# shaunliewsmu/ai-laryngeal-video-based-classifier

Measured on AMD Instinct MI355X. Metric: clips/sec fwd ViViT-B 32x224^2 bf16, higher is better.
Workload: dtype bf16; 1 GPU; ViViT-B/16x2 forward, 32x224x224 clips, batch 8 per GPU (BASELINE configs[1]); model=ViViT-B/16x2 (joint space-time, 12L, d768, 12H, 3137 tokens), global_batch=8, seq_len=3137, parallelism=dp1, streams=2, hip_graph=True

## Files before the change

ai-laryngeal-video-based-classifier_amd/csrc/attention.hip:

```cpp
#include "common.hpp"

#include <type_traits>

namespace vc {

constexpr int AK = 64;
constexpr int KV_TILE_BYTES = AK * 64 * 2;
constexpr int KV_SLOT = 2 * KV_TILE_BYTES;
constexpr int NSLOT = 4;
constexpr float LIM = 256.0f;

#ifndef VC_ATTN_SWEXP
#define VC_ATTN_SWEXP 0
#endif
__device__ __forceinline__ float sw_exp2(float x) {
    x = fmaxf(x, -126.0f);
    const float t = x + 12582912.0f;
    const float f = x - (t - 12582912.0f);
    float p = __builtin_fmaf(f, 0.0550292665f, 0.2422569819f);
    p = __builtin_fmaf(f, p, 0.6932530550f);
    p = __builtin_fmaf(f, p, 0.9999513387f);
    return __builtin_bit_cast(float, __builtin_bit_cast(unsigned, p) + (__builtin_bit_cast(unsigned, t) << 23));
}

__device__ __forceinline__ int kswz(int r, int c) { return c ^ ((r >> 1) & 7); }
__device__ __forceinline__ int vswz(int r, int c) { return c ^ (((r >> 1) & 1) << 2); }

__device__ __forceinline__ void adma16s(const void* sbase, uint32_t voff, uint32_t lds_addr) {
    asm volatile("s_mov_b32 m0, %2\n\ts_nop 0\n\tglobal_load_lds_dwordx4 %0, %1"
                 :
                 : "v"(voff), "s"(sbase), "s"(lds_addr)
                 : "memory", "m0");
}

template <int N>
__device__ __forceinline__ void attn_wait_vm() {
    static_assert(N >= 0 && N < 16, "vmcnt");
    __builtin_amdgcn_s_waitcnt(0x0F70 | N);
}

__device__ __forceinline__ void attn_sync() {
    __builtin_amdgcn_s_waitcnt(0xC07F);
    __builtin_amdgcn_s_barrier();
    asm volatile("" ::: "memory");
    __builtin_amdgcn_sched_barrier(0);
}

template <bool REBASE_ALWAYS, bool WLSE, int ET = VC_ELEM_BF16>
__global__ void __launch_bounds__(256, 2)
attn_fwd_d64_kernel(const uint16_t* __restrict__ qkv, int64_t ld, int S, int H, float c_log2,
                    uint16_t* __restrict__ out, int64_t ldo, float* __restrict__ lse) {
    constexpr int QB = 1;
    constexpr int AQ = 128;
    constexpr int NS = NSLOT;
    extern __shared__ __attribute__((aligned(16))) char smem[];

    const int nq = gridDim.x, nwg = gridDim.x * gridDim.y;
    const int L = blockIdx.y * nq + blockIdx.x;
    const int xq = nwg >> 3, xr = nwg & 7, xcd = L & 7;
    const int wg = (xcd < xr ? xcd * (xq + 1) : xr * (xq + 1) + (xcd - xr) * xq) + (L >> 3);
    const int qblk = wg % nq;
    const int bh = wg / nq;
    const int b = bh / H, hh = bh % H;
    const int tid = threadIdx.x, lane = tid & 63;
    const int wave = __builtin_amdgcn_readfirstlane(tid >> 6);
    const int r = lane & 31, h = lane >> 5;

    const int64_t tok0 = (int64_t)b * S;
    const uint16_t* qbase = qkv + hh * 64;
    const uint16_t* kbase = qkv + (int64_t)H * 64 + hh * 64 + tok0 * ld;
    const uint16_t* vbase = qkv + (int64_t)2 * H * 64 + hh * 64 + tok0 * ld;
    const uint32_t lds0 = __builtin_amdgcn_readfirstlane(
        (uint32_t)(uintptr_t)(const __attribute__((address_space(3))) char*)smem);

    v8s qf[QB][4];
#pragma unroll
    for (int qb = 0; qb < QB; ++qb) {
        const int q = qblk * AQ + (wave * QB + qb) * 32 + r;
        const int qc = q < S ? q : S - 1;
        const uint16_t* qrow = qbase + (tok0 + qc) * ld + 8 * h;
#pragma unroll
        for (int kk = 0; kk < 4; ++kk) {
            const v8s raw = *reinterpret_cast<const v8s*>(qrow + 16 * kk);
            if (c_log2 == 1.0f) {
                qf[qb][kk] = raw;
            } else {
#pragma unroll
                for (int j = 0; j < 8; ++j) qf[qb][kk][j] = (short)to16<ET>(from16<ET>((unsigned short)raw[j]) * c_log2);
            }
        }
    }

    const int srow = wave * 16 + (lane >> 3), spc = lane & 7;
    const uint32_t ko0 = (uint32_t)(srow * ld + kswz(srow, spc) * 8) * 2;
    const uint32_t ko1 = (uint32_t)((srow + 8) * ld + kswz(srow + 8, spc) * 8) * 2;
    const uint32_t vo0 = (uint32_t)(srow * ld + vswz(srow, spc) * 8) * 2;
    const uint32_t vo1 = (uint32_t)((srow + 8) * ld + vswz(srow + 8, spc) * 8) * 2;
    auto stage = [&](int t) {
        const uint32_t s = lds0 + (t % NS) * KV_SLOT + wave * 16 * 128;
        const uint16_t* kt = kbase + (int64_t)t * AK * ld;
        const uint16_t* vt = vbase + (int64_t)t * AK * ld;
        adma16s(kt, ko0, __builtin_amdgcn_readfirstlane(s));
        adma16s(kt, ko1, __builtin_amdgcn_readfirstlane(s + 8 * 128));
        adma16s(vt, vo0, __builtin_amdgcn_readfirstlane(s + KV_TILE_BYTES));
        adma16s(vt, vo1, __builtin_amdgcn_readfirstlane(s + KV_TILE_BYTES + 8 * 128));
    };

    int koff[4];
#pragma unroll
    for (int kk = 0; kk < 4; ++kk) koff[kk] = r * 128 + kswz(r, kk * 2 + h) * 16;
    const int gi = lane & 15;
    const int tq = gi >> 2, tp = gi & 3;
    const int gcol = ((lane >> 4) & 1) * 16 + tp * 4;
    int voff[2];
#pragma unroll
    for (int db = 0; db < 2; ++db) {
        const int col = db * 32 + gcol;
        const int ra = 4 * h + tq;
        voff[db] = KV_TILE_BYTES + ra * 128 + vswz(ra, col >> 3) * 16 + (col & 7) * 2;
    }

    v16f o[QB][2];
    v16f minit[QB];
    v2f l_run[QB];
    v4f lsum[QB];
    v8s sel;
    {
        const short one = ET == VC_ELEM_F16 ? (short)0x3C00 : (short)0x3F80;
        const short v = (((lane >> 4) & 1) == ((lane & 15) >> 3)) ? one : (short)0;
#pragma unroll
        for (int j = 0; j < 8; ++j) sel[j] = v;
    }

    auto qk_mfma = [&](const char* slot, v16f (&sc)[QB][2], bool kb1 = true) {
#pragma unroll
        for (int kk = 0; kk < 4; ++kk) {
            const v8s k0 = *reinterpret_cast<const v8s*>(slot + koff[kk]);
#pragma unroll
            for (int qb = 0; qb < QB; ++qb) sc[qb][0] = mfma32x16<ET>(k0, qf[qb][kk], kk == 0 ? minit[qb] : sc[qb][0]);
            if (kb1) {
                const v8s k1 = *reinterpret_cast<const v8s*>(slot + koff[kk] + 4096);
#pragma unroll
                for (int qb = 0; qb < QB; ++qb) sc[qb][1] = mfma32x16<ET>(k1, qf[qb][kk], kk == 0 ? minit[qb] : sc[qb][1]);
            }
        }
    };
    auto qk = [&](const char* slot, int t, v16f (&sc)[QB][2]) {
        const int kv0 = t * AK;
        if (kv0 + AK > S) {
            const bool kb1 = kv0 + 32 < S;
            qk_mfma(slot, sc, kb1);
#pragma unroll
            for (int qb = 0; qb < QB; ++qb)
#pragma unroll
                for (int e = 0; e < 16; ++e) {
                    const int key = (e & 3) + 8 * (e >> 2) + 4 * h;
                    if (kv0 + key >= S) sc[qb][0][e] = -INFINITY;
                    if (!kb1 || kv0 + 32 + key >= S) sc[qb][1][e] = -INFINITY;
                }
        } else {
            qk_mfma(slot, sc);
        }
    };
    auto exp_all = [&](v16f (&sc)[QB][2]) {
#pragma unroll
        for (int qb = 0; qb < QB; ++qb)
#pragma unroll
            for (int e = 0; e < 16; ++e) {
                sc[qb][0][e] = __builtin_amdgcn_exp2f(sc[qb][0][e]);
                sc[qb][1][e] = __builtin_amdgcn_exp2f(sc[qb][1][e]);
            }
    };
    auto psum = [&](const v16f (&sc)[QB][2], v2f (&ps)[QB]) {
#pragma unroll
        for (int qb = 0; qb < QB; ++qb) {
            v2f u[8];
#pragma unroll
            for (int j = 0; j < 4; ++j) {
                u[j] = v2f{sc[qb][0][4 * j], sc[qb][0][4 * j + 1]} + v2f{sc[qb][0][4 * j + 2], sc[qb][0][4 * j + 3]};
                u[4 + j] = v2f{sc[qb][1][4 * j], sc[qb][1][4 * j + 1]} + v2f{sc[qb][1][4 * j + 2], sc[qb][1][4 * j + 3]};
            }
            ps[qb] = ((u[0] + u[1]) + (u[2] + u[3])) + ((u[4] + u[5]) + (u[6] + u[7]));
        }
    };
    auto rowmax_of = [&](const v16f (&sc)[2]) {
        float m0 = fmaxf(sc[0][0], sc[1][0]), m1 = fmaxf(sc[0][1], sc[1][1]);
#pragma unroll
        for (int e = 2; e < 16; e += 2) {
            m0 = fmaxf(m0, fmaxf(sc[0][e], sc[1][e]));
            m1 = fmaxf(m1, fmaxf(sc[0][e + 1], sc[1][e + 1]));
        }
        const float m = fmaxf(m0, m1);
        return fmaxf(m, __shfl_xor(m, 32, 64));
    };
    auto rebase = [&](auto next_c, v16f (&sc)[QB][2], v16f (&sn)[QB][2]) {
        constexpr int NEXT = decltype(next_c)::value;
#pragma unroll
        for (int qb = 0; qb < QB; ++qb) {
            const float delta = fmaxf(rowmax_of(sc[qb]), 0.f);
            const float alpha = __builtin_amdgcn_exp2f(-delta);
#pragma unroll
            for (int e = 0; e < 16; ++e) {
                sc[qb][0][e] -= delta;
                sc[qb][1][e] -= delta;
                o[qb][0][e] *= alpha;
                o[qb][1][e] *= alpha;
                minit[qb][e] -= delta;
            }
            if constexpr (NEXT != 2) {
#pragma unroll
                for (int e = 0; e < 16; ++e) { sn[qb][0][e] -= delta; sn[qb][1][e] -= delta; }
            }
            if constexpr (WLSE) {
                l_run[qb] *= alpha;
            } else {
                lsum[qb] *= __shfl(alpha, (lane & 15) + ((lane >> 5) << 4), 64);
            }
        }
    };

    const int ntiles = (S + AK - 1) / AK;
    if ((L >> 8) & 1) __builtin_amdgcn_s_setprio(1);

    const bool live = qblk * AQ + wave * 32 < S;
    auto dead_pass = [&]() {
        stage(0);
        if (ntiles > 1) stage(1);
        if (ntiles > 2) stage(2);
        if (ntiles > 2) attn_wait_vm<4>();
        else attn_wait_vm<0>();
        attn_sync();
        for (int t = 0; t < ntiles; ++t) {
            if (t + NS - 1 < ntiles) stage(t + NS - 1);
            if (t + 2 < ntiles) {
                if (t + 3 < ntiles) attn_wait_vm<4>();
                else attn_wait_vm<0>();
                attn_sync();
            }
        }
    };
    auto pass = [&](auto rb_c) {
        constexpr bool RB = decltype(rb_c)::value;
#pragma unroll
        for (int qb = 0; qb < QB; ++qb) {
#pragma unroll
            for (int e = 0; e < 16; ++e) { o[qb][0][e] = 0.f; o[qb][1][e] = 0.f; minit[qb][e] = 0.f; }
            l_run[qb] = v2f{0.f, 0.f};
            lsum[qb] = v4f{0.f, 0.f, 0.f, 0.f};
        }
        if (!live) {
            dead_pass();
            return;
        }
        stage(0);
        if (ntiles > 1) stage(1);
        if (ntiles > 2) stage(2);
        if (ntiles > 2) attn_wait_vm<4>();
        else attn_wait_vm<0>();
        attn_sync();
        v16f scur[QB][2];
        qk(smem, 0, scur);
#pragma unroll
        for (int qb = 0; qb < QB; ++qb) {
            const float m = rowmax_of(scur[qb]);
#pragma unroll
            for (int e = 0; e < 16; ++e) { scur[qb][0][e] -= m; scur[qb][1][e] -= m; minit[qb][e] = -m; }
        }

        auto vread = [&](const char* slot, int g, v8s (&vv)[2]) {
#pragma unroll
            for (int db = 0; db < 2; ++db) {
                const char* pa = slot + voff[db] + g * 16 * 128;
                const v4s va = __builtin_amdgcn_ds_read_tr16_b64_v4i16((lds_v4s*)pa);
                const v4s vb = __builtin_amdgcn_ds_read_tr16_b64_v4i16((lds_v4s*)(pa + 8 * 128));
                vv[db][0] = va[0]; vv[db][1] = va[1]; vv[db][2] = va[2]; vv[db][3] = va[3];
                vv[db][4] = vb[0]; vv[db][5] = vb[1]; vv[db][6] = vb[2]; vv[db][7] = vb[3];
            }
        };
        auto iter = [&](auto next_c, const char* slot, const char* nslot, int t) {
            constexpr int NEXT = decltype(next_c)::value;
            constexpr bool FULLNEXT = NEXT == 0 || NEXT == 3;
            constexpr bool PIPE = !RB && FULLNEXT && QB == 1;
            if constexpr (NEXT == 3) stage(t + NS - 1);
            else if (t + NS - 1 < ntiles) stage(t + NS - 1);
            v16f snext[QB][2];
            v8s vcur[2], vnxt[2];
            if constexpr (PIPE) {
                auto ex = [&](int i) {
                    if (i < VC_ATTN_SWEXP) scur[0][i >> 4][i & 15] = sw_exp2(scur[0][i >> 4][i & 15]);
                    else scur[0][i >> 4][i & 15] = __builtin_amdgcn_exp2f(scur[0][i >> 4][i & 15]);
                };
                v8s ka = *reinterpret_cast<const v8s*>(nslot + koff[0]);
                v8s kb = *reinterpret_cast<const v8s*>(nslot + koff[0] + 4096);
                ex(0); ex(1); ex(2); ex(3);
                __builtin_amdgcn_sched_barrier(0);
#pragma unroll
                for (int kk = 0; kk < 4; ++kk) {
                    v8s na, nb;
                    if (kk < 3) {
                        na = *reinterpret_cast<const v8s*>(nslot + koff[kk + 1]);
                        nb = *reinterpret_cast<const v8s*>(nslot + koff[kk + 1] + 4096);
                    } else {
                        vread(slot, 0, vcur);
                    }
                    snext[0][0] = mfma32x16<ET>(ka, qf[0][kk], kk == 0 ? minit[0] : snext[0][0]);
                    ex(4 + 6 * kk); ex(5 + 6 * kk); ex(6 + 6 * kk);
                    snext[0][1] = mfma32x16<ET>(kb, qf[0][kk], kk == 0 ? minit[0] : snext[0][1]);
                    ex(7 + 6 * kk); ex(8 + 6 * kk); ex(9 + 6 * kk);
                    ka = na;
                    kb = nb;
                    __builtin_amdgcn_sched_barrier(0);
                }
                ex(28); ex(29); ex(30); ex(31);
            } else if constexpr (FULLNEXT) {
                qk_mfma(nslot, snext);
            } else if constexpr (NEXT == 1) {
                qk(nslot, t + 1, snext);
            }

            if constexpr (PIPE) {
                if constexpr (WLSE) {
                    v2f ps[QB];
                    psum(scur, ps);
                    if (__any(!(ps[0][0] + ps[0][1] <= LIM))) {
                        qk(slot, t, scur);
                        rebase(next_c, scur, snext);
                        exp_all(scur);
                        psum(scur, ps);
                    }
                    l_run[0] += ps[0];
                }
            } else if constexpr (WLSE) {
                v2f ps[QB];
                exp_all(scur);
                psum(scur, ps);
                bool grow = RB;
#pragma unroll
                for (int qb = 0; qb < QB; ++qb) grow = grow || !(ps[qb][0] + ps[qb][1] <= LIM);
                if (__any(grow)) {
                    qk(slot, t, scur);
                    rebase(next_c, scur, snext);
                    exp_all(scur);
                    psum(scur, ps);
                }
#pragma unroll
                for (int qb = 0; qb < QB; ++qb) l_run[qb] += ps[qb];
            } else {
                if constexpr (RB) rebase(next_c, scur, snext);
                exp_all(scur);
            }

            const bool pv_kb1 = NEXT != 2 || t * AK + 32 < S;
            if constexpr (PIPE) {
                auto pack = [&](int g) {
                    v4u pu;
#pragma unroll
                    for (int jj = 0; jj < 4; ++jj)
                        pu[jj] = pack2<ET>(scur[0][g >> 1][8 * (g & 1) + 2 * jj], scur[0][g >> 1][8 * (g & 1) + 2 * jj + 1]);
                    return __builtin_bit_cast(v8s, pu);
                };
                v8s pf = pack(0);
                __builtin_amdgcn_sched_barrier(0);
#pragma unroll
                for (int g = 0; g < 4; ++g) {
                    if (g < 3) vread(slot, g + 1, vnxt);
                    o[0][0] = mfma32x16<ET>(vcur[0], pf, o[0][0]);
                    o[0][1] = mfma32x16<ET>(vcur[1], pf, o[0][1]);
                    if constexpr (!WLSE) lsum[0] = mfma16x32<ET>(sel, pf, lsum[0]);
                    if (g < 3) {
                        pf = pack(g + 1);
                        vcur[0] = vnxt[0];
                        vcur[1] = vnxt[1];
                    }
                    __builtin_amdgcn_sched_barrier(0);
                }
            } else
#pragma unroll
            for (int kb = 0; kb < 2; ++kb)
#pragma unroll
                for (int s2 = 0; s2 < 2; ++s2) {
                    if (kb == 1 && !pv_kb1) continue;
                    v8s pf[QB];
#pragma unroll
                    for (int qb = 0; qb < QB; ++qb) {
                        v4u pu;
#pragma unroll
                        for (int jj = 0; jj < 4; ++jj)
                            pu[jj] = pack2<ET>(scur[qb][kb][8 * s2 + 2 * jj], scur[qb][kb][8 * s2 + 2 * jj + 1]);
                        pf[qb] = __builtin_bit_cast(v8s, pu);
                    }
#pragma unroll
                    for (int db = 0; db < 2; ++db) {
                        const char* pa = slot + voff[db] + (kb * 32 + 16 * s2) * 128;
                        v4s va = __builtin_amdgcn_ds_read_tr16_b64_v4i16((lds_v4s*)pa);
                        v4s vb = __builtin_amdgcn_ds_read_tr16_b64_v4i16((lds_v4s*)(pa + 8 * 128));
                        v8s vv;
                        vv[0] = va[0]; vv[1] = va[1]; vv[2] = va[2]; vv[3] = va[3];
                        vv[4] = vb[0]; vv[5] = vb[1]; vv[6] = vb[2]; vv[7] = vb[3];
#pragma unroll
                        for (int qb = 0; qb < QB; ++qb) o[qb][db] = mfma32x16<ET>(vv, pf[qb], o[qb][db]);
                    }
                    if constexpr (!WLSE) {
#pragma unroll
                        for (int qb = 0; qb < QB; ++qb) lsum[qb] = mfma16x32<ET>(sel, pf[qb], lsum[qb]);
                    }
                }

            if constexpr (NEXT == 3) {
                attn_wait_vm<4>();
                attn_sync();
            } else if (t + 2 < ntiles) {
                if (t + 3 < ntiles) attn_wait_vm<4>();
                else attn_wait_vm<0>();
                attn_sync();
            }
            if constexpr (NEXT != 2) {
#pragma unroll
                for (int qb = 0; qb < QB; ++qb) { scur[qb][0] = snext[qb][0]; scur[qb][1] = snext[qb][1]; }
            }
        };

        using full_c = std::integral_constant<int, 0>;
        using fast_c = std::integral_constant<int, 3>;
        const int nfull = S / AK;
        int t = 0;
        for (; t + 5 <= nfull && t + 6 < ntiles; t += NS) {
            iter(fast_c{}, smem + 0 * KV_SLOT, smem + 1 * KV_SLOT, t);
            iter(fast_c{}, smem + 1 * KV_SLOT, smem + 2 * KV_SLOT, t + 1);
            iter(fast_c{}, smem + 2 * KV_SLOT, smem + 3 * KV_SLOT, t + 2);
            iter(fast_c{}, smem + 3 * KV_SLOT, smem + 0 * KV_SLOT, t + 3);
        }
        for (; t + 5 <= nfull; t += NS) {
            iter(full_c{}, smem + 0 * KV_SLOT, smem + 1 * KV_SLOT, t);
            iter(full_c{}, smem + 1 * KV_SLOT, smem + 2 * KV_SLOT, t + 1);
            iter(full_c{}, smem + 2 * KV_SLOT, smem + 3 * KV_SLOT, t + 2);
            iter(full_c{}, smem + 3 * KV_SLOT, smem + 0 * KV_SLOT, t + 3);
        }
        for (; t < ntiles; ++t) {
            const char* slot = smem + (t % NS) * KV_SLOT;
            const char* nslot = smem + ((t + 1) % NS) * KV_SLOT;
            if (t + 1 < ntiles) iter(std::integral_constant<int, 1>{}, slot, nslot, t);
            else iter(std::integral_constant<int, 2>{}, slot, nslot, t);
        }
    };

    auto row_total = [&](int qb) {
        if constexpr (WLSE) {
            const float l_own = l_run[qb][0] + l_run[qb][1];
            return l_own + __shfl_xor(l_own, 32, 64);
        } else {
            return __shfl(lsum[qb][0], (r & 15) + ((r >> 4) << 5), 64);
        }
    };

    if constexpr (WLSE || REBASE_ALWAYS) {
        pass(std::integral_constant<bool, REBASE_ALWAYS>{});
    } else {
        pass(std::false_type{});
        bool bad = false;
#pragma unroll
        for (int qb = 0; qb < QB; ++qb) bad = bad || !(row_total(qb) <= 0x1p64f);
        if (__syncthreads_or(bad)) pass(std::true_type{});
    }

#pragma unroll
    for (int qb = 0; qb < QB; ++qb) {
        const int q = qblk * AQ + (wave * QB + qb) * 32 + r;
        const int qc = q < S ? q : S - 1;
        const float l_tot = row_total(qb);
        const float inv = 1.0f / l_tot;
        if constexpr (WLSE) {
            if (h == 0 && q < S) lse[(int64_t)bh * S + q] = -minit[qb][0] + __log2f(l_tot);
        }
        unsigned pk[2][4][2];
#pragma unroll
        for (int db = 0; db < 2; ++db)
#pragma unroll
            for (int g = 0; g < 4; ++g) {
                pk[db][g][0] = pack2<ET>(o[qb][db][4 * g + 0] * inv, o[qb][db][4 * g + 1] * inv);
                pk[db][g][1] = pack2<ET>(o[qb][db][4 * g + 2] * inv, o[qb][db][4 * g + 3] * inv);
            }
        uint16_t* orow = out + (tok0 + qc) * ldo + hh * 64;
#pragma unroll
        for (int db = 0; db < 2; ++db)
#pragma unroll
            for (int g = 0; g < 4; g += 2) {
                auto x0 = __builtin_amdgcn_permlane32_swap(pk[db][g][0], pk[db][g + 1][0], false, false);
                auto x1 = __builtin_amdgcn_permlane32_swap(pk[db][g][1], pk[db][g + 1][1], false, false);
                uint4 v;
                v.x = x0[0]; v.y = x1[0]; v.z = x0[1]; v.w = x1[1];
                if (q < S) *reinterpret_cast<uint4*>(orow + db * 32 + g * 8 + h * 8) = v;
            }
    }
}

template <bool REBASE_ALWAYS, bool WLSE, int ET = VC_ELEM_BF16>
static void launch_attn(const uint16_t* qkv, int64_t ld, int64_t B, int64_t S, int64_t H, float c_log2, uint16_t* out,
                        int64_t ldo, hipStream_t stream, float* lse = nullptr) {
    dim3 grid((unsigned)((S + 127) / 128), (unsigned)(B * H));
    attn_fwd_d64_kernel<REBASE_ALWAYS, WLSE, ET><<<grid, 256, NSLOT * KV_SLOT, stream>>>(qkv, ld, (int)S, (int)H, c_log2,
                                                                                   out, ldo, lse);
}

int launch_attn_short(const uint16_t* qkv, int64_t ld, int64_t B, int64_t S, int64_t H, float c_log2, uint16_t* out,
                      int64_t ldo, int elem, hipStream_t stream);
constexpr int64_t SHORT_MAX_S = 256;

}

using namespace vc;

static int attn_checks(const uint16_t* qkv, int64_t ld, int64_t B, int64_t S, int64_t H, int64_t head_dim,
                       const uint16_t* out, int64_t ldo) {
    if (!qkv || !out) return fail(VC_ERR_INVALID_ARG, "vc_attention_fwd: null pointer");
    if (head_dim != 64) return fail(VC_ERR_UNSUPPORTED, "vc_attention_fwd: head_dim must be 64");
    if (B <= 0 || S <= 0 || H <= 0 || ld < 3 * H * 64 || ldo < H * 64 || ld % 8 || ldo % 8)
        return fail(VC_ERR_INVALID_ARG, "vc_attention_fwd: bad shape / leading dimension");
    if ((((uintptr_t)qkv) | ((uintptr_t)out)) & 15)
        return fail(VC_ERR_INVALID_ARG, "vc_attention_fwd: pointers must be 16-byte aligned");
    if (B * H > 65535 || S > (1 << 24)) return fail(VC_ERR_INVALID_ARG, "vc_attention_fwd: grid too large");
    return 0;
}

extern "C" int vc_attention_fwd(const uint16_t* qkv, int64_t ld, int64_t B, int64_t S, int64_t H, int64_t head_dim,
                                float scale, int q_prescaled, uint16_t* out, int64_t ldo, hipStream_t stream) {
    if (int rc = attn_checks(qkv, ld, B, S, H, head_dim, out, ldo)) return rc;
    const float c_log2 = q_prescaled ? 1.0f : scale * 1.4426950408889634f;
    if (S <= SHORT_MAX_S) return launch_attn_short(qkv, ld, B, S, H, c_log2, out, ldo, VC_ELEM_BF16, stream);
    launch_attn<false, false>(qkv, ld, B, S, H, c_log2, out, ldo, stream);
    return check_launch("vc_attention_fwd");
}

extern "C" int vc_attention_fwd_h16(const uint16_t* qkv, int64_t ld, int64_t B, int64_t S, int64_t H,
                                    int64_t head_dim, float scale, int q_prescaled, int elem, uint16_t* out,
                                    int64_t ldo, hipStream_t stream) {
    if (int rc = attn_checks(qkv, ld, B, S, H, head_dim, out, ldo)) return rc;
    const float c_log2 = q_prescaled ? 1.0f : scale * 1.4426950408889634f;
    if (S <= SHORT_MAX_S && (elem == VC_ELEM_F16 || elem == VC_ELEM_BF16))
        return launch_attn_short(qkv, ld, B, S, H, c_log2, out, ldo, elem, stream);
    if (elem == VC_ELEM_F16) launch_attn<false, false, VC_ELEM_F16>(qkv, ld, B, S, H, c_log2, out, ldo, stream);
    else if (elem == VC_ELEM_BF16) launch_attn<false, false>(qkv, ld, B, S, H, c_log2, out, ldo, stream);
    else return fail(VC_ERR_INVALID_ARG, "vc_attention_fwd_h16: bad elem");
    return check_launch("vc_attention_fwd_h16");
}

extern "C" int vc_attention_fwd_lse(const uint16_t* qkv, int64_t ld, int64_t B, int64_t S, int64_t H, int64_t head_dim,
                                    float scale, int q_prescaled, uint16_t* out, int64_t ldo, float* lse,
                                    hipStream_t stream) {
    if (int rc = attn_checks(qkv, ld, B, S, H, head_dim, out, ldo)) return rc;
    if (!lse) return fail(VC_ERR_INVALID_ARG, "vc_attention_fwd_lse: null lse");
    const float c_log2 = q_prescaled ? 1.0f : scale * 1.4426950408889634f;
    launch_attn<false, true>(qkv, ld, B, S, H, c_log2, out, ldo, stream, lse);
    return check_launch("vc_attention_fwd_lse");
}

extern "C" int vc_attention_fwd_rebase_always(const uint16_t* qkv, int64_t ld, int64_t B, int64_t S, int64_t H,
                                              float scale, uint16_t* out, int64_t ldo, hipStream_t stream) {
    if (int rc = attn_checks(qkv, ld, B, S, H, 64, out, ldo)) return rc;
    launch_attn<true, false>(qkv, ld, B, S, H, scale * 1.4426950408889634f, out, ldo, stream);
    return check_launch("vc_attention_fwd_rebase_always");
}
```

Baseline: 1069 clips/s.

## Switch attention MFMA tiling from 32x32x16 to 16x16x32 with two query blocks

Rewrites the flash-attention inner loop to use 16x16x32 MFMA tiles, with each wave handling two 16-row query blocks instead of one 32-row block. The V LDS swizzle, the softmax row-max reduction (now an extra cross-lane shuffle), the row-sum accumulation via a ones-vector MFMA, and the output packing (permlane16 instead of permlane32) are all reworked to match. The software exp2 option is removed. The aim is better MFMA throughput and finer interleaving of exp work with matrix ops, at the cost of more instructions and extra shuffle reductions.

```diff
diff --git a/ai-laryngeal-video-based-classifier_amd/csrc/attention.hip b/ai-laryngeal-video-based-classifier_amd/csrc/attention.hip
--- a/ai-laryngeal-video-based-classifier_amd/csrc/attention.hip
+++ b/ai-laryngeal-video-based-classifier_amd/csrc/attention.hip
@@ -10,21 +10,8 @@
 constexpr int NSLOT = 4;
 constexpr float LIM = 256.0f;
 
-#ifndef VC_ATTN_SWEXP
-#define VC_ATTN_SWEXP 0
-#endif
-__device__ __forceinline__ float sw_exp2(float x) {
-    x = fmaxf(x, -126.0f);
-    const float t = x + 12582912.0f;
-    const float f = x - (t - 12582912.0f);
-    float p = __builtin_fmaf(f, 0.0550292665f, 0.2422569819f);
-    p = __builtin_fmaf(f, p, 0.6932530550f);
-    p = __builtin_fmaf(f, p, 0.9999513387f);
-    return __builtin_bit_cast(float, __builtin_bit_cast(unsigned, p) + (__builtin_bit_cast(unsigned, t) << 23));
-}
-
 __device__ __forceinline__ int kswz(int r, int c) { return c ^ ((r >> 1) & 7); }
-__device__ __forceinline__ int vswz(int r, int c) { return c ^ (((r >> 1) & 1) << 2); }
+__device__ __forceinline__ int vswz(int r, int c) { return c ^ (((r >> 1) & 3) << 1); }
 
 __device__ __forceinline__ void adma16s(const void* sbase, uint32_t voff, uint32_t lds_addr) {
     asm volatile("s_mov_b32 m0, %2\n\ts_nop 0\n\tglobal_load_lds_dwordx4 %0, %1"
@@ -46,11 +33,12 @@
     __builtin_amdgcn_sched_barrier(0);
 }
 
+__device__ __forceinline__ v4f splat4(float x) { return v4f{x, x, x, x}; }
+
 template <bool REBASE_ALWAYS, bool WLSE, int ET = VC_ELEM_BF16>
 __global__ void __launch_bounds__(256, 2)
 attn_fwd_d64_kernel(const uint16_t* __restrict__ qkv, int64_t ld, int S, int H, float c_log2,
                     uint16_t* __restrict__ out, int64_t ldo, float* __restrict__ lse) {
-    constexpr int QB = 1;
     constexpr int AQ = 128;
     constexpr int NS = NSLOT;
     extern __shared__ __attribute__((aligned(16))) char smem[];
@@ -64,7 +52,7 @@
     const int b = bh / H, hh = bh % H;
     const int tid = threadIdx.x, lane = tid & 63;
     const int wave = __builtin_amdgcn_readfirstlane(tid >> 6);
-    const int r = lane & 31, h = lane >> 5;
+    const int c = lane & 15, g = lane >> 4;
 
     const int64_t tok0 = (int64_t)b * S;
     const uint16_t* qbase = qkv + hh * 64;
@@ -73,20 +61,20 @@
     const uint32_t lds0 = __builtin_amdgcn_readfirstlane(
         (uint32_t)(uintptr_t)(const __attribute__((address_space(3))) char*)smem);
 
-    v8s qf[QB][4];
-#pragma unroll
-    for (int qb = 0; qb < QB; ++qb) {
-        const int q = qblk * AQ + (wave * QB + qb) * 32 + r;
+    v8s qf[2][2];
+#pragma unroll
+    for (int qb = 0; qb < 2; ++qb) {
+        const int q = qblk * AQ + wave * 32 + qb * 16 + c;
         const int qc = q < S ? q : S - 1;
-        const uint16_t* qrow = qbase + (tok0 + qc) * ld + 8 * h;
-#pragma unroll
-        for (int kk = 0; kk < 4; ++kk) {
-            const v8s raw = *reinterpret_cast<const v8s*>(qrow + 16 * kk);
+        const uint16_t* qrow = qbase + (tok0 + qc) * ld + 8 * g;
+#pragma unroll
+        for (int ks = 0; ks < 2; ++ks) {
+            const v8s raw = *reinterpret_cast<const v8s*>(qrow + 32 * ks);
             if (c_log2 == 1.0f) {
-                qf[qb][kk] = raw;
+                qf[qb][ks] = raw;
             } else {
 #pragma unroll
-                for (int j = 0; j < 8; ++j) qf[qb][kk][j] = (short)to16<ET>(from16<ET>((unsigned short)raw[j]) * c_log2);
+                for (int j = 0; j < 8; ++j) qf[qb][ks][j] = (short)to16<ET>(from16<ET>((unsigned short)raw[j]) * c_log2);
             }
         }
     }
@@ -106,116 +94,103 @@
         adma16s(vt, vo1, __builtin_amdgcn_readfirstlane(s + KV_TILE_BYTES + 8 * 128));
     };
 
-    int koff[4];
-#pragma unroll
-    for (int kk = 0; kk < 4; ++kk) koff[kk] = r * 128 + kswz(r, kk * 2 + h) * 16;
-    const int gi = lane & 15;
-    const int tq = gi >> 2, tp = gi & 3;
-    const int gcol = ((lane >> 4) & 1) * 16 + tp * 4;
-    int voff[2];
-#pragma unroll
-    for (int db = 0; db < 2; ++db) {
-        const int col = db * 32 + gcol;
-        const int ra = 4 * h + tq;
+    int koff[2];
+#pragma unroll
+    for (int ks = 0; ks < 2; ++ks) koff[ks] = c * 128 + kswz(c, ks * 4 + g) * 16;
+    const int tq = c >> 2, tp = c & 3;
+    int voff[4];
+#pragma unroll
+    for (int db = 0; db < 4; ++db) {
+        const int col = db * 16 + tp * 4;
+        const int ra = 4 * g + tq;
         voff[db] = KV_TILE_BYTES + ra * 128 + vswz(ra, col >> 3) * 16 + (col & 7) * 2;
     }
 
-    v16f o[QB][2];
-    v16f minit[QB];
-    v2f l_run[QB];
-    v4f lsum[QB];
-    v8s sel;
+    v4f o[2][4];
+    v4f minit[2];
+    v2f l_run[2];
+    v4f lsum[2];
+    v8s ones;
     {
         const short one = ET == VC_ELEM_F16 ? (short)0x3C00 : (short)0x3F80;
-        const short v = (((lane >> 4) & 1) == ((lane & 15) >> 3)) ? one : (short)0;
-#pragma unroll
-        for (int j = 0; j < 8; ++j) sel[j] = v;
+#pragma unroll
+        for (int j = 0; j < 8; ++j) ones[j] = one;
     }
 
-    auto qk_mfma = [&](const char* slot, v16f (&sc)[QB][2], bool kb1 = true) {
-#pragma unroll
-        for (int kk = 0; kk < 4; ++kk) {
-            const v8s k0 = *reinterpret_cast<const v8s*>(slot + koff[kk]);
-#pragma unroll
-            for (int qb = 0; qb < QB; ++qb) sc[qb][0] = mfma32x16<ET>(k0, qf[qb][kk], kk == 0 ? minit[qb] : sc[qb][0]);
-            if (kb1) {
-                const v8s k1 = *reinterpret_cast<const v8s*>(slot + koff[kk] + 4096);
-#pragma unroll
-                for (int qb = 0; qb < QB; ++qb) sc[qb][1] = mfma32x16<ET>(k1, qf[qb][kk], kk == 0 ? minit[qb] : sc[qb][1]);
-            }
-        }
-    };
-    auto qk = [&](const char* slot, int t, v16f (&sc)[QB][2]) {
+    auto qk_mfma = [&](const char* slot, v4f (&sc)[2][4], int nkb = 4) {
+#pragma unroll
+        for (int kb = 0; kb < 4; ++kb) {
+            if (kb < nkb) {
+                const v8s k0 = *reinterpret_cast<const v8s*>(slot + koff[0] + kb * 2048);
+                const v8s k1 = *reinterpret_cast<const v8s*>(slot + koff[1] + kb * 2048);
+#pragma unroll
+                for (int qb = 0; qb < 2; ++qb) sc[qb][kb] = mfma16x32<ET>(k1, qf[qb][1], minit[qb]);
+#pragma unroll
+                for (int qb = 0; qb < 2; ++qb) sc[qb][kb] = mfma16x32<ET>(k0, qf[qb][0], sc[qb][kb]);
+            } else {
+                sc[0][kb] = splat4(-INFINITY);
+                sc[1][kb] = splat4(-INFINITY);
+            }
+        }
+    };
+    auto qk = [&](const char* slot, int t, v4f (&sc)[2][4]) {
         const int kv0 = t * AK;
         if (kv0 + AK > S) {
-            const bool kb1 = kv0 + 32 < S;
-            qk_mfma(slot, sc, kb1);
-#pragma unroll
-            for (int qb = 0; qb < QB; ++qb)
-#pragma unroll
-                for (int e = 0; e < 16; ++e) {
-                    const int key = (e & 3) + 8 * (e >> 2) + 4 * h;
-                    if (kv0 + key >= S) sc[qb][0][e] = -INFINITY;
-                    if (!kb1 || kv0 + 32 + key >= S) sc[qb][1][e] = -INFINITY;
-                }
+            qk_mfma(slot, sc, (S - kv0 + 15) >> 4);
+#pragma unroll
+            for (int qb = 0; qb < 2; ++qb)
+#pragma unroll
+                for (int kb = 0; kb < 4; ++kb)
+#pragma unroll
+                    for (int e = 0; e < 4; ++e)
+                        if (kv0 + 16 * kb + 4 * g + e >= S) sc[qb][kb][e] = -INFINITY;
         } else {
             qk_mfma(slot, sc);
         }
     };
-    auto exp_all = [&](v16f (&sc)[QB][2]) {
-#pragma unroll
-        for (int qb = 0; qb < QB; ++qb)
-#pragma unroll
-            for (int e = 0; e < 16; ++e) {
-                sc[qb][0][e] = __builtin_amdgcn_exp2f(sc[qb][0][e]);
-                sc[qb][1][e] = __builtin_amdgcn_exp2f(sc[qb][1][e]);
-            }
-    };
-    auto psum = [&](const v16f (&sc)[QB][2], v2f (&ps)[QB]) {
-#pragma unroll
-        for (int qb = 0; qb < QB; ++qb) {
-            v2f u[8];
-#pragma unroll
-            for (int j = 0; j < 4; ++j) {
-                u[j] = v2f{sc[qb][0][4 * j], sc[qb][0][4 * j + 1]} + v2f{sc[qb][0][4 * j + 2], sc[qb][0][4 * j + 3]};
-                u[4 + j] = v2f{sc[qb][1][4 * j], sc[qb][1][4 * j + 1]} + v2f{sc[qb][1][4 * j + 2], sc[qb][1][4 * j + 3]};
-            }
-            ps[qb] = ((u[0] + u[1]) + (u[2] + u[3])) + ((u[4] + u[5]) + (u[6] + u[7]));
-        }
-    };
-    auto rowmax_of = [&](const v16f (&sc)[2]) {
-        float m0 = fmaxf(sc[0][0], sc[1][0]), m1 = fmaxf(sc[0][1], sc[1][1]);
-#pragma unroll
-        for (int e = 2; e < 16; e += 2) {
-            m0 = fmaxf(m0, fmaxf(sc[0][e], sc[1][e]));
-            m1 = fmaxf(m1, fmaxf(sc[0][e + 1], sc[1][e + 1]));
-        }
-        const float m = fmaxf(m0, m1);
+    auto exp_all = [&](v4f (&sc)[2][4]) {
+#pragma unroll
+        for (int qb = 0; qb < 2; ++qb)
+#pragma unroll
+            for (int kb = 0; kb < 4; ++kb)
+#pragma unroll
+                for (int e = 0; e < 4; ++e) sc[qb][kb][e] = __builtin_amdgcn_exp2f(sc[qb][kb][e]);
+    };
+    auto psum = [&](const v4f (&sc)[2][4], v2f (&ps)[2]) {
+#pragma unroll
+        for (int qb = 0; qb < 2; ++qb) {
+            v2f u[4];
+#pragma unroll
+            for (int kb = 0; kb < 4; ++kb) u[kb] = v2f{sc[qb][kb][0], sc[qb][kb][1]} + v2f{sc[qb][kb][2], sc[qb][kb][3]};
+            ps[qb] = (u[0] + u[1]) + (u[2] + u[3]);
+        }
+    };
+    auto rowmax_of = [&](const v4f (&sc)[4]) {
+        float m0 = fmaxf(sc[0][0], sc[0][1]), m1 = fmaxf(sc[0][2], sc[0][3]);
+#pragma unroll
+        for (int kb = 1; kb < 4; ++kb) {
+            m0 = fmaxf(m0, fmaxf(sc[kb][0], sc[kb][1]));
+            m1 = fmaxf(m1, fmaxf(sc[kb][2], sc[kb][3]));
+        }
+        float m = fmaxf(m0, m1);
+        m = fmaxf(m, __shfl_xor(m, 16, 64));
         return fmaxf(m, __shfl_xor(m, 32, 64));
     };
-    auto rebase = [&](auto next_c, v16f (&sc)[QB][2], v16f (&sn)[QB][2]) {
+    auto rebase = [&](auto next_c, v4f (&sc)[2][4], v4f (&sn)[2][4]) {
         constexpr int NEXT = decltype(next_c)::value;
 #pragma unroll
-        for (int qb = 0; qb < QB; ++qb) {
+        for (int qb = 0; qb < 2; ++qb) {
             const float delta = fmaxf(rowmax_of(sc[qb]), 0.f);
             const float alpha = __builtin_amdgcn_exp2f(-delta);
 #pragma unroll
-            for (int e = 0; e < 16; ++e) {
-                sc[qb][0][e] -= delta;
-                sc[qb][1][e] -= delta;
-                o[qb][0][e] *= alpha;
-                o[qb][1][e] *= alpha;
-                minit[qb][e] -= delta;
-            }
-            if constexpr (NEXT != 2) {
-#pragma unroll
-                for (int e = 0; e < 16; ++e) { sn[qb][0][e] -= delta; sn[qb][1][e] -= delta; }
-            }
-            if constexpr (WLSE) {
-                l_run[qb] *= alpha;
-            } else {
-                lsum[qb] *= __shfl(alpha, (lane & 15) + ((lane >> 5) << 4), 64);
-            }
+            for (int i = 0; i < 4; ++i) {
+                sc[qb][i] -= delta;
+                o[qb][i] *= alpha;
+                if constexpr (NEXT != 2) sn[qb][i] -= delta;
+            }
+            minit[qb] -= delta;
+            if constexpr (WLSE) l_run[qb] *= alpha;
+            else lsum[qb] *= alpha;
         }
     };
 
@@ -242,11 +217,12 @@
     auto pass = [&](auto rb_c) {
         constexpr bool RB = decltype(rb_c)::value;
 #pragma unroll
-        for (int qb = 0; qb < QB; ++qb) {
-#pragma unroll
-            for (int e = 0; e < 16; ++e) { o[qb][0][e] = 0.f; o[qb][1][e] = 0.f; minit[qb][e] = 0.f; }
+        for (int qb = 0; qb < 2; ++qb) {
+#pragma unroll
+            for (int db = 0; db < 4; ++db) o[qb][db] = splat4(0.f);
+            minit[qb] = splat4(0.f);
             l_run[qb] = v2f{0.f, 0.f};
-            lsum[qb] = v4f{0.f, 0.f, 0.f, 0.f};
+            lsum[qb] = splat4(0.f);
         }
         if (!live) {
             dead_pass();
@@ -258,60 +234,77 @@
         if (ntiles > 2) attn_wait_vm<4>();
         else attn_wait_vm<0>();
         attn_sync();
-        v16f scur[QB][2];
+        v4f scur[2][4];
         qk(smem, 0, scur);
 #pragma unroll
-        for (int qb = 0; qb < QB; ++qb) {
+        for (int qb = 0; qb < 2; ++qb) {
             const float m = rowmax_of(scur[qb]);
 #pragma unroll
-            for (int e = 0; e < 16; ++e) { scur[qb][0][e] -= m; scur[qb][1][e] -= m; minit[qb][e] = -m; }
-        }
-
-        auto vread = [&](const char* slot, int g, v8s (&vv)[2]) {
-#pragma unroll
-            for (int db = 0; db < 2; ++db) {
-                const char* pa = slot + voff[db] + g * 16 * 128;
-                const v4s va = __builtin_amdgcn_ds_read_tr16_b64_v4i16((lds_v4s*)pa);
-                const v4s vb = __builtin_amdgcn_ds_read_tr16_b64_v4i16((lds_v4s*)(pa + 8 * 128));
-                vv[db][0] = va[0]; vv[db][1] = va[1]; vv[db][2] = va[2]; vv[db][3] = va[3];
-                vv[db][4] = vb[0]; vv[db][5] = vb[1]; vv[db][6] = vb[2]; vv[db][7] = vb[3];
-            }
+            for (int kb = 0; kb < 4; ++kb) scur[qb][kb] -= m;
+            minit[qb] = splat4(-m);
+        }
+
+        auto vread = [&](const char* slot, int j, int db) {
+            const char* pa = slot + voff[db] + j * 32 * 128;
+            const v4s va = __builtin_amdgcn_ds_read_tr16_b64_v4i16((lds_v4s*)pa);
+            const v4s vb = __builtin_amdgcn_ds_read_tr16_b64_v4i16((lds_v4s*)(pa + 16 * 128));
+            v8s vv;
+            vv[0] = va[0]; vv[1] = va[1]; vv[2] = va[2]; vv[3] = va[3];
+            vv[4] = vb[0]; vv[5] = vb[1]; vv[6] = vb[2]; vv[7] = vb[3];
+            return vv;
+        };
+        auto pack = [&](const v4f (&sc)[2][4], int qb, int j) {
+            v4u pu;
+            pu[0] = pack2<ET>(sc[qb][2 * j][0], sc[qb][2 * j][1]);
+            pu[1] = pack2<ET>(sc[qb][2 * j][2], sc[qb][2 * j][3]);
+            pu[2] = pack2<ET>(sc[qb][2 * j + 1][0], sc[qb][2 * j + 1][1]);
+            pu[3] = pack2<ET>(sc[qb][2 * j + 1][2], sc[qb][2 * j + 1][3]);
+            return __builtin_bit_cast(v8s, pu);
         };
         auto iter = [&](auto next_c, const char* slot, const char* nslot, int t) {
             constexpr int NEXT = decltype(next_c)::value;
             constexpr bool FULLNEXT = NEXT == 0 || NEXT == 3;
-            constexpr bool PIPE = !RB && FULLNEXT && QB == 1;
+            constexpr bool PIPE = !RB && FULLNEXT;
             if constexpr (NEXT == 3) stage(t + NS - 1);
             else if (t + NS - 1 < ntiles) stage(t + NS - 1);
-            v16f snext[QB][2];
-            v8s vcur[2], vnxt[2];
+            v4f snext[2][4];
+            v8s vcur, pf[2];
             if constexpr (PIPE) {
                 auto ex = [&](int i) {
-                    if (i < VC_ATTN_SWEXP) scur[0][i >> 4][i & 15] = sw_exp2(scur[0][i >> 4][i & 15]);
-                    else scur[0][i >> 4][i & 15] = __builtin_amdgcn_exp2f(scur[0][i >> 4][i & 15]);
+                    scur[(i >> 2) & 1][i >> 3][i & 3] = __builtin_amdgcn_exp2f(scur[(i >> 2) & 1][i >> 3][i & 3]);
                 };
-                v8s ka = *reinterpret_cast<const v8s*>(nslot + koff[0]);
-                v8s kb = *reinterpret_cast<const v8s*>(nslot + koff[0] + 4096);
-                ex(0); ex(1); ex(2); ex(3);
+                v8s ka0 = *reinterpret_cast<const v8s*>(nslot + koff[0]);
+                v8s ka1 = *reinterpret_cast<const v8s*>(nslot + koff[1]);
+                ex(0); ex(1);
                 __builtin_amdgcn_sched_barrier(0);
 #pragma unroll
-                for (int kk = 0; kk < 4; ++kk) {
-                    v8s na, nb;
-                    if (kk < 3) {
-                        na = *reinterpret_cast<const v8s*>(nslot + koff[kk + 1]);
-                        nb = *reinterpret_cast<const v8s*>(nslot + koff[kk + 1] + 4096);
+                for (int kb = 0; kb < 4; ++kb) {
+                    v8s na0, na1;
+                    if (kb < 3) {
+                        na0 = *reinterpret_cast<const v8s*>(nslot + koff[0] + (kb + 1) * 2048);
+                        na1 = *reinterpret_cast<const v8s*>(nslot + koff[1] + (kb + 1) * 2048);
                     } else {
-                        vread(slot, 0, vcur);
-                    }
-                    snext[0][0] = mfma32x16<ET>(ka, qf[0][kk], kk == 0 ? minit[0] : snext[0][0]);
-                    ex(4 + 6 * kk); ex(5 + 6 * kk); ex(6 + 6 * kk);
-                    snext[0][1] = mfma32x16<ET>(kb, qf[0][kk], kk == 0 ? minit[0] : snext[0][1]);
-                    ex(7 + 6 * kk); ex(8 + 6 * kk); ex(9 + 6 * kk);
-                    ka = na;
-                    kb = nb;
+                        vcur = vread(slot, 0, 0);
+                    }
+                    snext[0][kb] = mfma16x32<ET>(ka1, qf[0][1], minit[0]);
+                    ex(2 + 6 * kb); ex(3 + 6 * kb);
+                    snext[1][kb] = mfma16x32<ET>(ka1, qf[1][1], minit[1]);
+                    ex(4 + 6 * kb);
+                    snext[0][kb] = mfma16x32<ET>(ka0, qf[0][0], snext[0][kb]);
+                    ex(5 + 6 * kb); ex(6 + 6 * kb);
+                    snext[1][kb] = mfma16x32<ET>(ka0, qf[1][0], snext[1][kb]);
+                    ex(7 + 6 * kb);
+                    if (kb == 3) {
+                        pf[0] = pack(scur, 0, 0);
+                        pf[1] = pack(scur, 1, 0);
+                    }
+                    ka0 = na0;
+                    ka1 = na1;
                     __builtin_amdgcn_sched_barrier(0);
                 }
-                ex(28); ex(29); ex(30); ex(31);
+                if constexpr (WLSE) {
+                    ex(26); ex(27); ex(28); ex(29); ex(30); ex(31);
+                }
             } else if constexpr (FULLNEXT) {
                 qk_mfma(nslot, snext);
             } else if constexpr (NEXT == 1) {
@@ -320,23 +313,26 @@
 
             if constexpr (PIPE) {
                 if constexpr (WLSE) {
-                    v2f ps[QB];
+                    v2f ps[2];
                     psum(scur, ps);
-                    if (__any(!(ps[0][0] + ps[0][1] <= LIM))) {
+                    if (__any(!(ps[0][0] + ps[0][1] <= LIM) || !(ps[1][0] + ps[1][1] <= LIM))) {
                         qk(slot, t, scur);
                         rebase(next_c, scur, snext);
                         exp_all(scur);
                         psum(scur, ps);
+                        pf[0] = pack(scur, 0, 0);
+                        pf[1] = pack(scur, 1, 0);
                     }
                     l_run[0] += ps[0];
+                    l_run[1] += ps[1];
                 }
             } else if constexpr (WLSE) {
-                v2f ps[QB];
+                v2f ps[2];
                 exp_all(scur);
                 psum(scur, ps);
                 bool grow = RB;
 #pragma unroll
-                for (int qb = 0; qb < QB; ++qb) grow = grow || !(ps[qb][0] + ps[qb][1] <= LIM);
+                for (int qb = 0; qb < 2; ++qb) grow = grow || !(ps[qb][0] + ps[qb][1] <= LIM);
                 if (__any(grow)) {
                     qk(slot, t, scur);
                     rebase(next_c, scur, snext);
@@ -344,67 +340,62 @@
                     psum(scur, ps);
                 }
 #pragma unroll
-                for (int qb = 0; qb < QB; ++qb) l_run[qb] += ps[qb];
+                for (int qb = 0; qb < 2; ++qb) l_run[qb] += ps[qb];
             } else {
                 if constexpr (RB) rebase(next_c, scur, snext);
                 exp_all(scur);
             }
 
-            const bool pv_kb1 = NEXT != 2 || t * AK + 32 < S;
             if constexpr (PIPE) {
-                auto pack = [&](int g) {
-                    v4u pu;
-#pragma unroll
-                    for (int jj = 0; jj < 4; ++jj)
-                        pu[jj] = pack2<ET>(scur[0][g >> 1][8 * (g & 1) + 2 * jj], scur[0][g >> 1][8 * (g & 1) + 2 * jj + 1]);
-                    return __builtin_bit_cast(v8s, pu);
+                auto ex = [&](int i) {
+                    scur[(i >> 2) & 1][i >> 3][i & 3] = __builtin_amdgcn_exp2f(scur[(i >> 2) & 1][i >> 3][i & 3]);
                 };
-                v8s pf = pack(0);
+                v8s pn[2];
                 __builtin_amdgcn_sched_barrier(0);
 #pragma unroll
-                for (int g = 0; g < 4; ++g) {
-                    if (g < 3) vread(slot, g + 1, vnxt);
-                    o[0][0] = mfma32x16<ET>(vcur[0], pf, o[0][0]);
-                    o[0][1] = mfma32x16<ET>(vcur[1], pf, o[0][1]);
-                    if constexpr (!WLSE) lsum[0] = mfma16x32<ET>(sel, pf, lsum[0]);
-                    if (g < 3) {
-                        pf = pack(g + 1);
-                        vcur[0] = vnxt[0];
-                        vcur[1] = vnxt[1];
-                    }
+                for (int s = 0; s < 8; ++s) {
+                    const int j = s >> 2, db = s & 3;
+                    v8s vnxt;
+                    if (s < 7) vnxt = vread(slot, (s + 1) >> 2, (s + 1) & 3);
+                    o[0][db] = mfma16x32<ET>(vcur, pf[0], o[0][db]);
+                    if constexpr (!WLSE) {
+                        if (s == 0) { ex(26); ex(27); }
+                        if (s == 1) { ex(29); ex(30); }
+                    }
+                    o[1][db] = mfma16x32<ET>(vcur, pf[1], o[1][db]);
+                    if constexpr (!WLSE) {
+                        if (s == 0) ex(28);
+                        if (s == 1) ex(31);
+                        if (db < 2) lsum[db] = mfma16x32<ET>(ones, pf[db], lsum[db]);
+                    }
+                    if (s == 2) pn[0] = pack(scur, 0, 1);
+                    if (s == 3) {
+                        pn[1] = pack(scur, 1, 1);
+                        pf[0] = pn[0];
+                        pf[1] = pn[1];
+                    }
+                    vcur = vnxt;
                     __builtin_amdgcn_sched_barrier(0);
                 }
-            } else
-#pragma unroll
-            for (int kb = 0; kb < 2; ++kb)
-#pragma unroll
-                for (int s2 = 0; s2 < 2; ++s2) {
-                    if (kb == 1 && !pv_kb1) continue;
-                    v8s pf[QB];
-#pragma unroll
-                    for (int qb = 0; qb < QB; ++qb) {
-                        v4u pu;
-#pragma unroll
-                        for (int jj = 0; jj < 4; ++jj)
-                            pu[jj] = pack2<ET>(scur[qb][kb][8 * s2 + 2 * jj], scur[qb][kb][8 * s2 + 2 * jj + 1]);
-                        pf[qb] = __builtin_bit_cast(v8s, pu);
-                    }
-#pragma unroll
-                    for (int db = 0; db < 2; ++db) {
-                        const char* pa = slot + voff[db] + (kb * 32 + 16 * s2) * 128;
-                        v4s va = __builtin_amdgcn_ds_read_tr16_b64_v4i16((lds_v4s*)pa);
-                        v4s vb = __builtin_amdgcn_ds_read_tr16_b64_v4i16((lds_v4s*)(pa + 8 * 128));
-                        v8s vv;
-                        vv[0] = va[0]; vv[1] = va[1]; vv[2] = va[2]; vv[3] = va[3];
-                        vv[4] = vb[0]; vv[5] = vb[1]; vv[6] = vb[2]; vv[7] = vb[3];
-#pragma unroll
-                        for (int qb = 0; qb < QB; ++qb) o[qb][db] = mfma32x16<ET>(vv, pf[qb], o[qb][db]);
+            } else {
+                const bool pv_j1 = NEXT != 2 || t * AK + 32 < S;
+#pragma unroll
+                for (int j = 0; j < 2; ++j) {
+                    if (j == 1 && !pv_j1) continue;
+                    pf[0] = pack(scur, 0, j);
+                    pf[1] = pack(scur, 1, j);
+#pragma unroll
+                    for (int db = 0; db < 4; ++db) {
+                        const v8s vv = vread(slot, j, db);
+                        o[0][db] = mfma16x32<ET>(vv, pf[0], o[0][db]);
+                        o[1][db] = mfma16x32<ET>(vv, pf[1], o[1][db]);
                     }
                     if constexpr (!WLSE) {
-#pragma unroll
-                        for (int qb = 0; qb < QB; ++qb) lsum[qb] = mfma16x32<ET>(sel, pf[qb], lsum[qb]);
+                        lsum[0] = mfma16x32<ET>(ones, pf[0], lsum[0]);
+                        lsum[1] = mfma16x32<ET>(ones, pf[1], lsum[1]);
                     }
                 }
+            }
 
             if constexpr (NEXT == 3) {
                 attn_wait_vm<4>();
@@ -416,7 +407,9 @@
             }
             if constexpr (NEXT != 2) {
 #pragma unroll
-                for (int qb = 0; qb < QB; ++qb) { scur[qb][0] = snext[qb][0]; scur[qb][1] = snext[qb][1]; }
+                for (int qb = 0; qb < 2; ++qb)
+#pragma unroll
+                    for (int kb = 0; kb < 4; ++kb) scur[qb][kb] = snext[qb][kb];
             }
         };
 
@@ -446,10 +439,11 @@
 
     auto row_total = [&](int qb) {
         if constexpr (WLSE) {
-            const float l_own = l_run[qb][0] + l_run[qb][1];
+            float l_own = l_run[qb][0] + l_run[qb][1];
+            l_own += __shfl_xor(l_own, 16, 64);
             return l_own + __shfl_xor(l_own, 32, 64);
         } else {
-            return __shfl(lsum[qb][0], (r & 15) + ((r >> 4) << 5), 64);
+            return lsum[qb][0];
         }
     };
 
@@ -459,38 +453,34 @@
         pass(std::false_type{});
         bool bad = false;
 #pragma unroll
-        for (int qb = 0; qb < QB; ++qb) bad = bad || !(row_total(qb) <= 0x1p64f);
+        for (int qb = 0; qb < 2; ++qb) bad = bad || !(row_total(qb) <= 0x1p64f);
         if (__syncthreads_or(bad)) pass(std::true_type{});
     }
 
 #pragma unroll
-    for (int qb = 0; qb < QB; ++qb) {
-        const int q = qblk * AQ + (wave * QB + qb) * 32 + r;
+    for (int qb = 0; qb < 2; ++qb) {
+        const int q = qblk * AQ + wave * 32 + qb * 16 + c;
         const int qc = q < S ? q : S - 1;
         const float l_tot = row_total(qb);
         const float inv = 1.0f / l_tot;
         if constexpr (WLSE) {
-            if (h == 0 && q < S) lse[(int64_t)bh * S + q] = -minit[qb][0] + __log2f(l_tot);
-        }
-        unsigned pk[2][4][2];
-#pragma unroll
-        for (int db = 0; db < 2; ++db)
-#pragma unroll
-            for (int g = 0; g < 4; ++g) {
-                pk[db][g][0] = pack2<ET>(o[qb][db][4 * g + 0] * inv, o[qb][db][4 * g + 1] * inv);
-                pk[db][g][1] = pack2<ET>(o[qb][db][4 * g + 2] * inv, o[qb][db][4 * g + 3] * inv);
-            }
+            if (g == 0 && q < S) lse[(int64_t)bh * S + q] = -minit[qb][0] + __log2f(l_tot);
+        }
         uint16_t* orow = out + (tok0 + qc) * ldo + hh * 64;
 #pragma unroll
-        for (int db = 0; db < 2; ++db)
-#pragma unroll
-            for (int g = 0; g < 4; g += 2) {
-                auto x0 = __builtin_amdgcn_permlane32_swap(pk[db][g][0], pk[db][g + 1][0], false, false);
-                auto x1 = __builtin_amdgcn_permlane32_swap(pk[db][g][1], pk[db][g + 1][1], false, false);
-                uint4 v;
-                v.x = x0[0]; v.y = x1[0]; v.z = x0[1]; v.w = x1[1];
-                if (q < S) *reinterpret_cast<uint4*>(orow + db * 32 + g * 8 + h * 8) = v;
-            }
+        for (int jp = 0; jp < 2; ++jp) {
+            unsigned pk[2][2];
+#pragma unroll
+            for (int s = 0; s < 2; ++s) {
+                pk[s][0] = pack2<ET>(o[qb][2 * jp + s][0] * inv, o[qb][2 * jp + s][1] * inv);
+                pk[s][1] = pack2<ET>(o[qb][2 * jp + s][2] * inv, o[qb][2 * jp + s][3] * inv);
+            }
+            auto x0 = __builtin_amdgcn_permlane16_swap(pk[0][0], pk[1][0], false, false);
+            auto x1 = __builtin_amdgcn_permlane16_swap(pk[0][1], pk[1][1], false, false);
+            uint4 v;
+            v.x = x0[0]; v.y = x1[0]; v.z = x0[1]; v.w = x1[1];
+            if (q < S) *reinterpret_cast<uint4*>(orow + (2 * jp + (g & 1)) * 16 + 4 * (g & 2)) = v;
+        }
     }
 }
 
```

Result: no change. 1059 clips/s (median of 2 runs) (-0.9%).
